# esi-neuroscience/syncopy

Hardware: AMD Instinct MI355X
Metric: trials/sec for mtmfft+coherence (256 ch x 4096 samples, 7 DPSS tapers, full CSD) (higher is better)
Workload: dtype f32 transforms; CSD operands fp16 hi+lo (22-bit), f32 accumulate; 1 GPU; BASELINE configs[2]: connectivityanalysis method='coh', AR(2) AnalogData, 256 ch x 4096 samp x 1000 trials per GPU, tapsmofrq=1 Hz (7 DPSS tapers), polyremoval=0, output='abs', inputs resident in HBM; trials_per_gpu=1000, channels=256, samples=4096, tapers=7, freqs=2049, batch=1000, fft_kernel=mtmfft_quad_kernel<12, 2, 2, false> + seq_mean_kernel

## Files before the change

### syncopy_amd/csrc/csdh.hip

```cpp
#include "spy_common.h"
#include "csd_args.h"
#include "csdh_kernel.h"
#include "csdh_launch.h"

namespace spycsd {

int csdh_run(hipStream_t stream, const float2* spec, long long nrows, int F, float2* acc, const float* absmax, int* flags, int f0,
             int nf, bool phase_exact) {
    if (nf <= 0 || nrows <= 0) return 0;
    if (nrows > 0x7fffffffLL) { spy::set_error("csd_accumulate: more than 2^31 - 1 rows in one call"); return -1; }
    CsdhArgs a{};
    a.spec = spec; a.nrows = nrows; a.F = F; a.acc = acc; a.absmax = absmax; a.flags = flags; a.f0 = f0; a.nf = nf;
    a.rs = (long long)F * 256; a.fs = 256;
    SPY_HIP_CHECK(hipFuncSetAttribute(reinterpret_cast<const void*>(csdh_kernel), hipFuncAttributeMaxDynamicSharedMemorySize,
                                      CSDH_LDS_BYTES));
    hipLaunchKernelGGL(csdh_kernel, dim3((unsigned)nf), dim3(512), CSDH_LDS_BYTES, stream, a);
    SPY_HIP_CHECK(hipGetLastError());
    CsdArgs b{};
    b.spec = spec; b.nrows = nrows; b.F = F; b.C = 256; b.acc = acc;
    b.nt = 8; b.ntiles = M3_TILES_PER_F; b.nitems = (long long)F * M3_TILES_PER_F; b.cpad = 256;
    b.item_base = (long long)f0 * M3_TILES_PER_F; b.item_end = (long long)(f0 + nf) * M3_TILES_PER_F;
    b.only_flagged = flags;
    if (phase_exact) {
        auto k = csd3m_kernel<256, 8, true, false, true>;
        SPY_HIP_CHECK(hipFuncSetAttribute(reinterpret_cast<const void*>(k), hipFuncAttributeMaxDynamicSharedMemorySize, M3_LDS_BYTES));
        hipLaunchKernelGGL(k, dim3((unsigned)nf), dim3(512), M3_LDS_BYTES, stream, b);
    } else {
        auto k = csd3m_kernel<256, 8, true, false, false>;
        SPY_HIP_CHECK(hipFuncSetAttribute(reinterpret_cast<const void*>(k), hipFuncAttributeMaxDynamicSharedMemorySize, M3_LDS_BYTES));
        hipLaunchKernelGGL(k, dim3((unsigned)nf), dim3(512), M3_LDS_BYTES, stream, b);
    }
    SPY_HIP_CHECK(hipGetLastError());
    return 0;
}

int csdh_absmax(hipStream_t stream, const float2* spec, long long nvalues, int nchan, float* absmax) {
    if (nvalues <= 0) return 0;
    if (nchan & 1 || nchan > 512 || 512 % nchan != 0) { spy::set_error("csd range pass: %d channels", nchan); return -1; }
    hipLaunchKernelGGL(csdh_absmax_kernel, dim3(2048), dim3(256), 0, stream, reinterpret_cast<const float4*>(spec), nvalues / 2, nchan,
                       reinterpret_cast<unsigned*>(absmax));
    SPY_HIP_CHECK(hipGetLastError());
    return 0;
}

}
```

### syncopy_amd/csrc/csdh_kernel.h

```cpp
#pragma once
#include "csd3m_kernel.h"

#ifndef CSDH_FENCE
#define CSDH_FENCE 0x78f
#endif
#ifndef CSDH_S1
#define CSDH_S1 7
#define CSDH_S2 15
#endif

#ifndef CSDH_ABL
#define CSDH_ABL 0
#endif

#ifdef CSDH_STAMPS
#define CSDH_STAMP(k) do { if (blockIdx.x == 0 && c >= 20 && c < 24) { asm volatile("s_waitcnt lgkmcnt(0)" ::: "memory"); \
        const unsigned long long t__ = __builtin_readcyclecounter(); \
        if (lane == 0) a.stamps[((c - 20) * 8 + G) * 8 + (k)] = t__; } } while (0)
#else
#define CSDH_STAMP(k) do { } while (0)
#endif

namespace spycsd {

typedef _Float16 f16x8 __attribute__((ext_vector_type(8)));
typedef float f32x2 __attribute__((ext_vector_type(2)));

struct CsdhArgs {
    const float2* spec;
    long long nrows;
    int F;
    float2* acc;
    const float* absmax;
    int* flags;
    int f0;
    int nf;
    unsigned long long* stamps;
    long long rs, fs;
};

constexpr int CSDH_PLANE = 16 * 1024;
constexpr int CSDH_BUF = 4 * CSDH_PLANE;
constexpr int CSDH_LDS_BYTES = 2 * CSDH_BUF + 1024 + 16;
constexpr int CSDH_KROWS = 32;

template <int NT_ = 17>
struct HTabT {
    static constexpr int NT = NT_, ND = 2;
    struct Gen { int ta[8][NT], tb[8][NT]; };
    static constexpr Gen make() {
        constexpr int SQR[6] = {8, 8, 12, 12, 4, 12}, SQC[6] = {0, 4, 0, 4, 0, 8};
        constexpr int DG[8] = {0, 10, 2, 14, 6, 8, 4, 12};
        Gen g{};
        int n[8] = {};
        for (int w = 0; w < 6; ++w)
            for (int r = SQR[w]; r < SQR[w] + 4; ++r)
                for (int c = SQC[w]; c < SQC[w] + 4; ++c) {
                    const int o = (r == SQR[w] && c == SQC[w] + 3) ? 6 + (w & 1) : w;
                    g.ta[o][n[o]] = r; g.tb[o][n[o]] = c; ++n[o];
                }
        for (int w = 6; w < 8; ++w)
            for (int b = 8 * (w - 6); b < 8 * (w - 6) + 8; b += 4)
                for (int r = b; r < b + 4; ++r)
                    for (int c = b; c < r; ++c) { g.ta[w][n[w]] = r; g.tb[w][n[w]] = c; ++n[w]; }
        for (int w = 0; w < 8; ++w)
            for (int d = DG[w]; d < DG[w] + 2; ++d) { g.ta[w][n[w]] = d; g.tb[w][n[w]] = d; ++n[w]; }
        return g;
    }
    static constexpr Gen T = make();
    static constexpr int ta(int g, int t) { return T.ta[g][t]; }
    static constexpr int tb(int g, int t) { return T.tb[g][t]; }
    static constexpr bool diag(int g, int t) { return T.ta[g][t] == T.tb[g][t]; }
    static constexpr int didx(int g, int t) {
        int d = 0;
        for (int u = 0; u < t; ++u) d += diag(g, u) ? 1 : 0;
        return d;
    }
    static constexpr bool complete() {
        int seen[16][16] = {};
        for (int w = 0; w < 8; ++w) {
            int nd = 0;
            for (int t = 0; t < NT; ++t) {
                if (T.ta[w][t] < T.tb[w][t] || T.ta[w][t] > 15 || T.tb[w][t] < 0) return false;
                ++seen[T.ta[w][t]][T.tb[w][t]];
                nd += diag(w, t) ? 1 : 0;
            }
            if (nd != ND) return false;
        }
        for (int r = 0; r < 16; ++r)
            for (int c = 0; c <= r; ++c)
                if (seen[r][c] != 1) return false;
        return true;
    }
};
using HTab = HTabT<>;
static_assert(HTab::complete(), "the deal of K4h's sub-tiles");
static_assert(HTab::NT == M3Tab<256>::NT, "17 sub-tiles per wave in either deal");

template <int G>
struct HPlan {
    using TAB = HTab;
    static constexpr int NT = TAB::NT;
    struct P {
        int tile[NT];
        int ablk[NT], bblk[NT];
        int aslot[NT], bslot[NT];
        bool aload[NT], bload[NT];
        bool diag[NT], dinb[NT];
    };
    static constexpr bool column_only(int x) {
        bool col = false;
        for (int t = 0; t < NT; ++t) {
            if (TAB::diag(G, t)) continue;
            if (TAB::ta(G, t) == x) return false;
            col = col || TAB::tb(G, t) == x;
        }
        return col;
    }
    static constexpr P make() {
        P p{};
        int key[NT] = {};
        for (int t = 0; t < NT; ++t) {
            p.tile[t] = t;
            key[t] = (TAB::tb(G, t) >> 1) * 256 + TAB::ta(G, t) * 16 + TAB::tb(G, t);
        }
        for (int i = 1; i < NT; ++i)
            for (int j = i; j > 0 && key[j] < key[j - 1]; --j) {
                int k = key[j]; key[j] = key[j - 1]; key[j - 1] = k;
                int u = p.tile[j]; p.tile[j] = p.tile[j - 1]; p.tile[j - 1] = u;
            }
        int ac[2] = {-1, -1}, bc[2] = {-1, -1};
        int alast = 1, blast = 1;
        for (int s = 0; s < NT; ++s) {
            const int t = p.tile[s];
            const int x = TAB::ta(G, t), y = TAB::tb(G, t);
            p.ablk[s] = x;
            p.bblk[s] = y;
            p.diag[s] = x == y;
            p.dinb[s] = x == y && column_only(x);
            p.aslot[s] = alast; p.aload[s] = false;
            p.bslot[s] = blast; p.bload[s] = false;
            if (!p.dinb[s]) {
                if (ac[0] == x) { p.aslot[s] = 0; }
                else if (ac[1] == x) { p.aslot[s] = 1; }
                else { p.aslot[s] = 1 - alast; p.aload[s] = true; ac[1 - alast] = x; }
                alast = p.aslot[s];
            }
            if (!p.diag[s] || p.dinb[s]) {
                if (bc[0] == y) { p.bslot[s] = 0; }
                else if (bc[1] == y) { p.bslot[s] = 1; }
                else { p.bslot[s] = 1 - blast; p.bload[s] = true; bc[1 - blast] = y; }
                blast = p.bslot[s];
            }
        }
        return p;
    }
    static constexpr P T = make();
};

__device__ __forceinline__ int csdh_exponent(float absmax) {
    const int e = (int)((__float_as_uint(absmax) >> 23) & 0xffu);
    int k = 141 - e;
    return k > 127 ? 127 : k;
}

__device__ __forceinline__ void csdh_tile(const f16x8 (&X)[4], const f16x8 (&Y)[4], f32x4& re, f32x4& im) {
    __builtin_amdgcn_s_setprio(1);
    im = __builtin_amdgcn_mfma_f32_16x16x32_f16(X[2], Y[0], im, 0, 0, 0);
    im = __builtin_amdgcn_mfma_f32_16x16x32_f16(X[2], Y[1], im, 0, 0, 0);
    im = __builtin_amdgcn_mfma_f32_16x16x32_f16(X[3], Y[0], im, 0, 0, 0);
    re = __builtin_amdgcn_mfma_f32_16x16x32_f16(X[0], Y[0], re, 0, 0, 0);
    re = __builtin_amdgcn_mfma_f32_16x16x32_f16(X[0], Y[1], re, 0, 0, 0);
    re = __builtin_amdgcn_mfma_f32_16x16x32_f16(X[1], Y[0], re, 0, 0, 0);
    re = __builtin_amdgcn_mfma_f32_16x16x32_f16(X[2], Y[2], re, 0, 0, 0);
    re = __builtin_amdgcn_mfma_f32_16x16x32_f16(X[2], Y[3], re, 0, 0, 0);
    re = __builtin_amdgcn_mfma_f32_16x16x32_f16(X[3], Y[2], re, 0, 0, 0);
    if (!(CSDH_ABL & 32)) im = -im;
    im = __builtin_amdgcn_mfma_f32_16x16x32_f16(X[0], Y[2], im, 0, 0, 0);
    im = __builtin_amdgcn_mfma_f32_16x16x32_f16(X[0], Y[3], im, 0, 0, 0);
    im = __builtin_amdgcn_mfma_f32_16x16x32_f16(X[1], Y[2], im, 0, 0, 0);
    __builtin_amdgcn_s_setprio(0);
}

__device__ __forceinline__ void csdh_diag_tile(const f16x8 (&X)[4], f32x4& s, f32x4& p, f32x4& m) {
    __builtin_amdgcn_s_setprio(1);
    m = __builtin_amdgcn_mfma_f32_16x16x32_f16(X[2], X[0], m, 0, 0, 0);
    m = __builtin_amdgcn_mfma_f32_16x16x32_f16(X[2], X[1], m, 0, 0, 0);
    m = __builtin_amdgcn_mfma_f32_16x16x32_f16(X[3], X[0], m, 0, 0, 0);
    s = __builtin_amdgcn_mfma_f32_16x16x32_f16(X[0], X[0], s, 0, 0, 0);
    s = __builtin_amdgcn_mfma_f32_16x16x32_f16(X[2], X[2], s, 0, 0, 0);
    p = __builtin_amdgcn_mfma_f32_16x16x32_f16(X[0], X[1], p, 0, 0, 0);
    p = __builtin_amdgcn_mfma_f32_16x16x32_f16(X[2], X[3], p, 0, 0, 0);
    if (!(CSDH_ABL & 32)) m = -m;
    __builtin_amdgcn_s_setprio(0);
}

template <int G, int s>
__device__ __forceinline__ void csdh_step(const f16x8 (&A)[2][4], const f16x8 (&B)[2][4], f32x4 (&re)[HTab::NT], f32x4 (&im)[HTab::NT],
                                          f32x4 (&pd)[HTab::ND]) {
    using PL = HPlan<G>;
    constexpr int t = PL::T.tile[s];
    if constexpr (PL::T.diag[s]) {
        const f16x8(&X)[4] = PL::T.dinb[s] ? B[PL::T.bslot[s]] : A[PL::T.aslot[s]];
        csdh_diag_tile(X, re[t], pd[HTab::didx(G, t)], im[t]);
    } else {
        csdh_tile(A[PL::T.aslot[s]], B[PL::T.bslot[s]], re[t], im[t]);
    }
}

template <int G>
__device__ __forceinline__ void csdh_fold_diagonal(f32x4 (&re)[HTab::NT], f32x4 (&im)[HTab::NT], f32x4 (&pd)[HTab::ND], float* ts,
                                                   int lane) {
    const int l15 = lane & 15, lq = lane >> 4;
    auto transposed = [&](const f32x4& v) {
#pragma unroll
        for (int r = 0; r < 4; ++r) ts[(4 * lq + r) * 17 + l15] = v[r];
        __builtin_amdgcn_fence(__ATOMIC_RELEASE, "wavefront");
        __builtin_amdgcn_wave_barrier();
        __builtin_amdgcn_fence(__ATOMIC_ACQUIRE, "wavefront");
        f32x4 o;
#pragma unroll
        for (int r = 0; r < 4; ++r) o[r] = ts[l15 * 17 + 4 * lq + r];
        __builtin_amdgcn_fence(__ATOMIC_RELEASE, "wavefront");
        __builtin_amdgcn_wave_barrier();
        __builtin_amdgcn_fence(__ATOMIC_ACQUIRE, "wavefront");
        return o;
    };
    m3_for<0, HTab::NT>([&](auto tc) {
        constexpr int t = decltype(tc)::value;
        if constexpr (HTab::diag(G, t)) {
            constexpr int d = HTab::didx(G, t);
            const f32x4 st = transposed(re[t]), pt = transposed(pd[d]), mt = transposed(im[t]);
#pragma unroll
            for (int r = 0; r < 4; ++r) {
                re[t][r] = 0.5f * (re[t][r] + st[r]) + (pd[d][r] + pt[r]);
                im[t][r] = im[t][r] - mt[r];
            }
        }
    });
}

template <int G, class KEXP>
__device__ __forceinline__ void csdh_finish(const CsdhArgs& a, f32x4 (&re)[HTab::NT], f32x4 (&im)[HTab::NT], f32x4 (&pd)[HTab::ND],
                                            float* ts, int nchunk, int f, int lane, int* vword, KEXP kexp) {
    using TAB = HTab;
    constexpr int NT = TAB::NT;
    const int l15 = lane & 15, lq = lane >> 4;
    const long long nrows = a.nrows;
    csdh_fold_diagonal<G>(re, im, pd, ts, lane);
    const float isign = (nchunk & 1) ? -1.f : 1.f;

    {
        const float floor2 = (float)nrows * 0.015625f;
        bool bad = false;
        m3_for<0, NT>([&](auto tc) {
            constexpr int t = decltype(tc)::value;
            if constexpr (TAB::diag(G, t)) {
                const bool dead = a.absmax[TAB::ta(G, t) * 16 + l15] == 0.f;
#pragma unroll
                for (int r = 0; r < 4; ++r)
                    if (4 * lq + r == l15) {
                        const float v = re[t][r];
                        bad = bad || !((v >= floor2 && v < __builtin_inff()) || (v == 0.f && dead));
                    }
            }
        });
        if (__any(bad) && lane == 0) *vword = 0;
    }
    __syncthreads();
    const bool valid = *vword != 0;
    if (a.flags && G == 0 && lane == 0) a.flags[f] = valid ? 0 : 1;
    if (!valid) return;

    m3_for<0, NT>([&](auto tc) {
        constexpr int t = decltype(tc)::value;
        constexpr int bi = TAB::ta(G, t), bj = TAB::tb(G, t);
        static_assert(bi >= bj, "a sub-tile lies on or below the diagonal");
        float2* const pb = a.acc + (size_t)f * 65536 + (size_t)(bi * 16 + 4 * lq) * 256 + bj * 16 + l15;
        const int kj = kexp(bj * 16 + l15);
        float2 old[4];
#pragma unroll
        for (int r = 0; r < 4; ++r) old[r] = pb[(size_t)r * 256];
#pragma unroll
        for (int r = 0; r < 4; ++r) {
            const int kk = -(kexp(bi * 16 + 4 * lq + r) + kj);
            pb[(size_t)r * 256] = make_float2(old[r].x + ldexpf(re[t][r], kk), old[r].y + ldexpf(isign * im[t][r], kk));
        }
    });
}

template <int G>
__device__ __forceinline__ void csdh_wave(const CsdhArgs& a, char* lds, int f, int lane) {
    using TAB = HTab;
    using PL = HPlan<G>;
    constexpr int NT = TAB::NT, ND = TAB::ND;
    constexpr int KG = G >> 1, CHH = G & 1;
    const int l15 = lane & 15, lq = lane >> 4;
    int* const kexp = reinterpret_cast<int*>(lds + 2 * CSDH_BUF);
    int* const vword = reinterpret_cast<int*>(lds + 2 * CSDH_BUF + 1024);

    const int lc0 = 128 * CHH + lane, lc1 = lc0 + 64;
    const int k0 = csdh_exponent(a.absmax[lc0]), k1 = csdh_exponent(a.absmax[lc1]);
    const float s0 = __uint_as_float((unsigned)(k0 + 127) << 23), s1 = __uint_as_float((unsigned)(k1 + 127) << 23);
    if (KG == 0) { kexp[lc0] = k0; kexp[lc1] = k1; }
    if (G == 0 && lane == 0) *vword = 1;

    const long long nrows = a.nrows;
    const int nchunk = (int)((nrows + CSDH_KROWS - 1) / CSDH_KROWS);
    const size_t rowstride = (size_t)a.rs;

    f32x2 st[8];
    const int nrows_i = (int)nrows;
    const int nfull = nrows_i / CSDH_KROWS;
    const char* const gb = reinterpret_cast<const char*>(a.spec) + ((size_t)f * a.fs + 128 * CHH) * 8;
    const size_t rowbytes = rowstride * 8;
    const unsigned voff = (unsigned)lane * 8u;
    const char* nextp = gb + (size_t)(CSDH_KROWS + 8 * KG) * rowbytes;
    auto fetch = [&](int c, int ph) {
        if (c < nfull) {
#pragma unroll
            for (int i = 0; i < 8; ++i) {
                if (CSDH_ABL & 1) st[i] = f32x2{(float)(i + lane), (float)(c - lane)};
                else if ((CSDH_ABL & 128) && c > 2) asm volatile("" : "+v"(st[i]));
                else {
                    typedef const __attribute__((address_space(1))) char gchar;
                    typedef const __attribute__((address_space(1))) f32x2 gf32x2;
                    gchar* rowp = (gchar*)(nextp + i * rowbytes);
                    asm("" : "+s"(rowp));
                    st[i] = *(gf32x2*)(rowp + voff + 512 * ph);
                }
            }
        } else {
            const int r0 = c * CSDH_KROWS + 8 * KG;
#pragma unroll
            for (int i = 0; i < 8; ++i) {
                const int r = min(r0 + i, nrows_i - 1);
                st[i] = *reinterpret_cast<const f32x2*>(gb + (size_t)r * rowbytes + 512 * ph + voff);
            }
        }
    };
    auto split2 = [](float x0, float x1, float s, unsigned& hi, unsigned& lo) {
        asm("v_fma_mixlo_f16 %0, %2, %4, 0\n\t"
            "v_fma_mixhi_f16 %0, %3, %4, 0\n\t"
            "v_fma_mixlo_f16 %1, %2, %4, -%0 op_sel_hi:[0,0,1]\n\t"
            "v_fma_mixhi_f16 %1, %3, %4, -%0 op_sel:[0,0,1] op_sel_hi:[0,0,1]"
            : "=&v"(hi), "=&v"(lo)
            : "v"(x0), "v"(x1), "v"(s));
    };
    typedef unsigned u32x4 __attribute__((ext_vector_type(4)));
    auto convert = [&](int c, int ph) {
        const float sc = ph ? s1 : s0;
        u32x4 rh, rl, ih, il;
        if (CSDH_ABL & 2) {
#pragma unroll
            for (int i = 0; i < 4; ++i) { rh[i] = rl[i] = __float_as_uint(st[2 * i][0]); ih[i] = il[i] = __float_as_uint(st[2 * i + 1][1]); }
        } else if (c < nfull) {
#pragma unroll
            for (int i = 0; i < 4; ++i) {
                unsigned h, l;
                split2(st[2 * i][0], st[2 * i + 1][0], sc, h, l);
                rh[i] = h; rl[i] = l;
                split2(st[2 * i][1], st[2 * i + 1][1], sc, h, l);
                ih[i] = h; il[i] = l;
            }
        } else {
            const int r0 = c * CSDH_KROWS + 8 * KG;
#pragma unroll
            for (int i = 0; i < 4; ++i) {
                const float sa = (r0 + 2 * i < nrows_i) ? sc : 0.f, sb = (r0 + 2 * i + 1 < nrows_i) ? sc : 0.f;
                unsigned h0, l0, h1, l1;
                split2(st[2 * i][0], st[2 * i][1], sa, h0, l0);
                split2(st[2 * i + 1][0], st[2 * i + 1][1], sb, h1, l1);
                rh[i] = (h0 & 0xffffu) | (h1 << 16);
                rl[i] = (l0 & 0xffffu) | (l1 << 16);
                ih[i] = (h0 >> 16) | (h1 & 0xffff0000u);
                il[i] = (l0 >> 16) | (l1 & 0xffff0000u);
            }
        }
        const int odd = c & 1;
        char* const w = lds + odd * CSDH_BUF + KG * 4096 + (lc0 + 64 * ph) * 16;
        char* const wr = w + (odd ? 2 * CSDH_PLANE : 0);
        char* const wi = w + (odd ? 0 : 2 * CSDH_PLANE);
        if (CSDH_ABL & 4) {
            if (rh[0] + rl[1] + ih[2] + il[3] == 123456u) *reinterpret_cast<u32x4*>(wr) = rh;
            return;
        }
        *reinterpret_cast<u32x4*>(wr) = rh;
        *reinterpret_cast<u32x4*>(wr + CSDH_PLANE) = rl;
        *reinterpret_cast<u32x4*>(wi) = ih;
        *reinterpret_cast<u32x4*>(wi + CSDH_PLANE) = il;
    };

    f32x4 re[NT], im[NT], pd[ND];
#pragma unroll
    for (int t = 0; t < NT; ++t)
#pragma unroll
        for (int r = 0; r < 4; ++r) { re[t][r] = 0.f; im[t][r] = 0.f; }
#pragma unroll
    for (int d = 0; d < ND; ++d)
#pragma unroll
        for (int r = 0; r < 4; ++r) pd[d][r] = 0.f;

    nextp -= (size_t)CSDH_KROWS * rowbytes;
    fetch(0, 0);
    convert(0, 0);
    fetch(0, 1);
    convert(0, 1);
    nextp += (size_t)CSDH_KROWS * rowbytes;
    __syncthreads();

    f16x8 A[2][4], B[2][4];
    unsigned rb = (unsigned)(lq * 4096 + l15 * 16);
    bool nofrag = false;
    auto ldfrag = [&](f16x8 (&dst)[4], int blk) {
#pragma unroll
        for (int p = 0; p < 4; ++p) {
            if (CSDH_ABL & 8) {
                asm volatile("" : "+v"(dst[p]));
                continue;
            }
            if ((CSDH_ABL & 64) && nofrag) continue;
            dst[p] = *reinterpret_cast<const f16x8*>(lds + rb + p * CSDH_PLANE + blk * 256);
        }
    };
    constexpr int S1 = CSDH_S1, S2 = CSDH_S2;

    for (int c = 0; c < nchunk; ++c) {
        CSDH_STAMP(0);
        if constexpr (PL::T.aload[0]) ldfrag(A[PL::T.aslot[0]], PL::T.ablk[0]);
        if constexpr (PL::T.bload[0]) ldfrag(B[PL::T.bslot[0]], PL::T.bblk[0]);
        fetch(c + 1, 0);
        __builtin_amdgcn_sched_barrier(CSDH_FENCE);
        m3_for<0, NT>([&](auto sc) {
            constexpr int s = decltype(sc)::value;
            if constexpr (s + 1 < NT) {
                if constexpr (PL::T.aload[s + 1]) ldfrag(A[PL::T.aslot[s + 1]], PL::T.ablk[s + 1]);
                if constexpr (PL::T.bload[s + 1]) ldfrag(B[PL::T.bslot[s + 1]], PL::T.bblk[s + 1]);
            }
            csdh_step<G, s>(A, B, re, im, pd);
            if constexpr (s == S1) {
                CSDH_STAMP(2);
#ifdef CSDH_STAMPS
                asm volatile("s_waitcnt vmcnt(0)" ::: "memory");
#endif
                CSDH_STAMP(3);
                convert(c + 1, 0);
                fetch(c + 1, 1);
                __builtin_amdgcn_sched_barrier(CSDH_FENCE);
                CSDH_STAMP(4);
            }
            if constexpr (s == 0) CSDH_STAMP(1);
            if constexpr (s == S2) {
                CSDH_STAMP(5);
#ifdef CSDH_STAMPS
                asm volatile("s_waitcnt vmcnt(0)" ::: "memory");
#endif
                CSDH_STAMP(6);
                convert(c + 1, 1);
            }
        });
        CSDH_STAMP(7);
        if (!(CSDH_ABL & 16)) __syncthreads();
        if (CSDH_ABL & 64) nofrag = true;
        rb ^= (unsigned)CSDH_BUF;
        nextp += (size_t)CSDH_KROWS * rowbytes;
    }

    csdh_finish<G>(a, re, im, pd, reinterpret_cast<float*>(lds + G * 2048), nchunk, f, lane, vword, [&](int ch) { return kexp[ch]; });
}

template <int G0, int G1>
__device__ __forceinline__ void csdh_dispatch(int g, const CsdhArgs& a, char* lds, int f, int lane) {
    if constexpr (G0 + 1 == G1) {
        csdh_wave<G0>(a, lds, f, lane);
    } else {
        constexpr int GM = (G0 + G1) / 2;
        if (g < GM) csdh_dispatch<G0, GM>(g, a, lds, f, lane);
        else csdh_dispatch<GM, G1>(g, a, lds, f, lane);
    }
}

__global__ void __launch_bounds__(512) SPY_M3_KATTR(8) csdh_kernel(CsdhArgs a) {
    SPY_DYN_SMEM(char, lds);
    const int tid = threadIdx.x;
    const int lane = tid & 63;
    const int wave = __builtin_amdgcn_readfirstlane(tid >> 6);
    const int f = a.f0 + (int)blockIdx.x;
    csdh_dispatch<0, 8>(wave, a, lds, f, lane);
}

__global__ void __launch_bounds__(256) csdh_absmax_kernel(const float4* __restrict__ spec, long long nquads, int C,
                                                          unsigned* __restrict__ out) {
    __shared__ unsigned sm[512];
    for (int i = threadIdx.x; i < 512; i += 256) sm[i] = 0u;
    __syncthreads();
    const long long per = C / 2;
    const long long stride = (long long)gridDim.x * 256;
    float m0 = 0.f, m1 = 0.f;
    long long q = (long long)blockIdx.x * 256 + threadIdx.x;
    const int cp = (int)(q % per);
    for (; q < nquads; q += stride) {
        const float4 v = spec[q];
        m0 = fmaxf(m0, fmaxf(fabsf(v.x), fabsf(v.y)));
        m1 = fmaxf(m1, fmaxf(fabsf(v.z), fabsf(v.w)));
    }
    atomicMax(&sm[2 * cp], __float_as_uint(m0));
    atomicMax(&sm[2 * cp + 1], __float_as_uint(m1));
    __syncthreads();
    for (int i = threadIdx.x; i < C; i += 256)
        if (sm[i]) atomicMax(&out[i], sm[i]);
}

}
```

Before: 51450 trials/s.

## Split CSD waves into heavy MFMA waves and loader waves with interleaved conversion

The sub-tile deal across the 8 waves changes. Four heavy waves now run only MFMA sub-tiles (22 each) at raised priority. The other four waves take fewer sub-tiles plus the diagonal blocks, and they also do all global fetches and fp16 hi/lo conversion, which are split into small pieces and interleaved between individual MFMAs. The fetch uses 16-byte vector loads with deeper prefetch (two chunks ahead), so spectra must now be 16-byte aligned. The aim is to keep the matrix pipes busy in some waves while the load and convert latency is hidden in the others, at the cost of load imbalance and higher register pressure in the loader waves.

```diff
diff --git a/syncopy_amd/csrc/csdh.hip b/syncopy_amd/csrc/csdh.hip
--- a/syncopy_amd/csrc/csdh.hip
+++ b/syncopy_amd/csrc/csdh.hip
@@ -9,6 +9,7 @@
              int nf, bool phase_exact) {
     if (nf <= 0 || nrows <= 0) return 0;
     if (nrows > 0x7fffffffLL) { spy::set_error("csd_accumulate: more than 2^31 - 1 rows in one call"); return -1; }
+    if (reinterpret_cast<uintptr_t>(spec) & 15u) { spy::set_error("csd_accumulate: 256-channel spectra must be 16-byte aligned"); return -1; }
     CsdhArgs a{};
     a.spec = spec; a.nrows = nrows; a.F = F; a.acc = acc; a.absmax = absmax; a.flags = flags; a.f0 = f0; a.nf = nf;
     a.rs = (long long)F * 256; a.fs = 256;
diff --git a/syncopy_amd/csrc/csdh_kernel.h b/syncopy_amd/csrc/csdh_kernel.h
--- a/syncopy_amd/csrc/csdh_kernel.h
+++ b/syncopy_amd/csrc/csdh_kernel.h
@@ -4,9 +4,14 @@
 #ifndef CSDH_FENCE
 #define CSDH_FENCE 0x78f
 #endif
-#ifndef CSDH_S1
-#define CSDH_S1 7
-#define CSDH_S2 15
+#ifndef CSDH_NH
+#define CSDH_NH 22
+#endif
+#ifndef CSDH_HEAVY_HI
+#define CSDH_HEAVY_HI 0
+#endif
+#ifndef CSDH_PRIO
+#define CSDH_PRIO 1
 #endif
 
 #ifndef CSDH_ABL
@@ -17,7 +22,10 @@
 #define CSDH_STAMP(k) do { if (blockIdx.x == 0 && c >= 20 && c < 24) { asm volatile("s_waitcnt lgkmcnt(0)" ::: "memory"); \
         const unsigned long long t__ = __builtin_readcyclecounter(); \
         if (lane == 0) a.stamps[((c - 20) * 8 + G) * 8 + (k)] = t__; } } while (0)
+#define CSDH_STAMP_HWID() do { if (blockIdx.x == 0 && lane == 0) \
+        a.stamps[256 + G] = __builtin_amdgcn_s_getreg(4 | (31 << 11)); } while (0)
 #else
+#define CSDH_STAMP_HWID() do { } while (0)
 #define CSDH_STAMP(k) do { } while (0)
 #endif
 
@@ -44,27 +52,36 @@
 constexpr int CSDH_LDS_BYTES = 2 * CSDH_BUF + 1024 + 16;
 constexpr int CSDH_KROWS = 32;
 
-template <int NT_ = 17>
+template <int NH_ = CSDH_NH>
 struct HTabT {
-    static constexpr int NT = NT_, ND = 2;
-    struct Gen { int ta[8][NT], tb[8][NT]; };
+    static constexpr int NH = NH_, NLO = 30 - NH_, NDL = 4;
+    static constexpr int NTMAX = NH > NLO + NDL ? NH : NLO + NDL;
+    static_assert(NH >= 17 && NH <= 24 && (96 - 4 * NH) % 4 == 0, "the heavy runs come out of the 96 full-row sub-tiles");
+    static constexpr bool heavy(int g) { return CSDH_HEAVY_HI ? g >= 4 : g < 4; }
+    static constexpr int idx(int g) { return g & 3; }
+    static constexpr int nt(int g) { return heavy(g) ? NH : NLO + NDL; }
+    static constexpr int nd(int g) { return heavy(g) ? 0 : NDL; }
+    struct Gen { int ta[8][NTMAX], tb[8][NTMAX]; };
     static constexpr Gen make() {
-        constexpr int SQR[6] = {8, 8, 12, 12, 4, 12}, SQC[6] = {0, 4, 0, 4, 0, 8};
-        constexpr int DG[8] = {0, 10, 2, 14, 6, 8, 4, 12};
+        int sr[96] = {}, sc[96] = {};
+        int m = 0;
+        for (int s = 0; s < 3; ++s)
+            for (int r = 4 * (s + 1); r < 16; ++r)
+                for (int c = 4 * s; c < 4 * s + 4; ++c) { sr[m] = r; sc[m] = c; ++m; }
         Gen g{};
-        int n[8] = {};
-        for (int w = 0; w < 6; ++w)
-            for (int r = SQR[w]; r < SQR[w] + 4; ++r)
-                for (int c = SQC[w]; c < SQC[w] + 4; ++c) {
-                    const int o = (r == SQR[w] && c == SQC[w] + 3) ? 6 + (w & 1) : w;
-                    g.ta[o][n[o]] = r; g.tb[o][n[o]] = c; ++n[o];
-                }
-        for (int w = 6; w < 8; ++w)
-            for (int b = 8 * (w - 6); b < 8 * (w - 6) + 8; b += 4)
-                for (int r = b; r < b + 4; ++r)
-                    for (int c = b; c < r; ++c) { g.ta[w][n[w]] = r; g.tb[w][n[w]] = c; ++n[w]; }
-        for (int w = 0; w < 8; ++w)
-            for (int d = DG[w]; d < DG[w] + 2; ++d) { g.ta[w][n[w]] = d; g.tb[w][n[w]] = d; ++n[w]; }
+        constexpr int per = (96 - 4 * NH) / 4;
+        for (int w = 0; w < 8; ++w) {
+            const int i = idx(w);
+            int n = 0;
+            if (heavy(w)) {
+                for (int k = 0; k < NH; ++k) { g.ta[w][n] = sr[i * NH + k]; g.tb[w][n] = sc[i * NH + k]; ++n; }
+            } else {
+                for (int k = 0; k < per; ++k) { g.ta[w][n] = sr[4 * NH + i * per + k]; g.tb[w][n] = sc[4 * NH + i * per + k]; ++n; }
+                for (int r = 4 * i; r < 4 * i + 4; ++r)
+                    for (int c = 4 * i; c < r; ++c) { g.ta[w][n] = r; g.tb[w][n] = c; ++n; }
+                for (int d = 4 * i; d < 4 * i + 4; ++d) { g.ta[w][n] = d; g.tb[w][n] = d; ++n; }
+            }
+        }
         return g;
     }
     static constexpr Gen T = make();
@@ -79,13 +96,14 @@
     static constexpr bool complete() {
         int seen[16][16] = {};
         for (int w = 0; w < 8; ++w) {
-            int nd = 0;
-            for (int t = 0; t < NT; ++t) {
+            int nd_ = 0;
+            for (int t = 0; t < nt(w); ++t) {
                 if (T.ta[w][t] < T.tb[w][t] || T.ta[w][t] > 15 || T.tb[w][t] < 0) return false;
                 ++seen[T.ta[w][t]][T.tb[w][t]];
-                nd += diag(w, t) ? 1 : 0;
-            }
-            if (nd != ND) return false;
+                nd_ += diag(w, t) ? 1 : 0;
+            }
+            if (nd_ != nd(w)) return false;
+            if (w < 4 && heavy(w) == heavy(w + 4)) return false;
         }
         for (int r = 0; r < 16; ++r)
             for (int c = 0; c <= r; ++c)
@@ -95,12 +113,11 @@
 };
 using HTab = HTabT<>;
 static_assert(HTab::complete(), "the deal of K4h's sub-tiles");
-static_assert(HTab::NT == M3Tab<256>::NT, "17 sub-tiles per wave in either deal");
 
 template <int G>
 struct HPlan {
     using TAB = HTab;
-    static constexpr int NT = TAB::NT;
+    static constexpr int NT = TAB::nt(G);
     struct P {
         int tile[NT];
         int ablk[NT], bblk[NT];
@@ -164,53 +181,68 @@
     return k > 127 ? 127 : k;
 }
 
-__device__ __forceinline__ void csdh_tile(const f16x8 (&X)[4], const f16x8 (&Y)[4], f32x4& re, f32x4& im) {
-    __builtin_amdgcn_s_setprio(1);
+__device__ __forceinline__ void csdh_tile_begin() { __builtin_amdgcn_sched_barrier(0); if (!CSDH_PRIO) __builtin_amdgcn_s_setprio(1); }
+__device__ __forceinline__ void csdh_tile_end() { if (!CSDH_PRIO) __builtin_amdgcn_s_setprio(0); __builtin_amdgcn_sched_barrier(0); }
+struct CsdhNoWork { __device__ __forceinline__ void operator()(int) const {} };
+
+template <class W>
+__device__ __forceinline__ void csdh_tile(const f16x8 (&X)[4], const f16x8 (&Y)[4], f32x4& re, f32x4& im, W&& work) {
+    csdh_tile_begin();
     im = __builtin_amdgcn_mfma_f32_16x16x32_f16(X[2], Y[0], im, 0, 0, 0);
+    work(0);
     im = __builtin_amdgcn_mfma_f32_16x16x32_f16(X[2], Y[1], im, 0, 0, 0);
     im = __builtin_amdgcn_mfma_f32_16x16x32_f16(X[3], Y[0], im, 0, 0, 0);
     re = __builtin_amdgcn_mfma_f32_16x16x32_f16(X[0], Y[0], re, 0, 0, 0);
+    work(1);
     re = __builtin_amdgcn_mfma_f32_16x16x32_f16(X[0], Y[1], re, 0, 0, 0);
     re = __builtin_amdgcn_mfma_f32_16x16x32_f16(X[1], Y[0], re, 0, 0, 0);
     re = __builtin_amdgcn_mfma_f32_16x16x32_f16(X[2], Y[2], re, 0, 0, 0);
+    work(2);
     re = __builtin_amdgcn_mfma_f32_16x16x32_f16(X[2], Y[3], re, 0, 0, 0);
     re = __builtin_amdgcn_mfma_f32_16x16x32_f16(X[3], Y[2], re, 0, 0, 0);
     if (!(CSDH_ABL & 32)) im = -im;
     im = __builtin_amdgcn_mfma_f32_16x16x32_f16(X[0], Y[2], im, 0, 0, 0);
+    work(3);
     im = __builtin_amdgcn_mfma_f32_16x16x32_f16(X[0], Y[3], im, 0, 0, 0);
     im = __builtin_amdgcn_mfma_f32_16x16x32_f16(X[1], Y[2], im, 0, 0, 0);
-    __builtin_amdgcn_s_setprio(0);
-}
-
-__device__ __forceinline__ void csdh_diag_tile(const f16x8 (&X)[4], f32x4& s, f32x4& p, f32x4& m) {
-    __builtin_amdgcn_s_setprio(1);
+    csdh_tile_end();
+}
+
+template <class W>
+__device__ __forceinline__ void csdh_diag_tile(const f16x8 (&X)[4], f32x4& s, f32x4& p, f32x4& m, W&& work) {
+    csdh_tile_begin();
     m = __builtin_amdgcn_mfma_f32_16x16x32_f16(X[2], X[0], m, 0, 0, 0);
+    work(0);
     m = __builtin_amdgcn_mfma_f32_16x16x32_f16(X[2], X[1], m, 0, 0, 0);
     m = __builtin_amdgcn_mfma_f32_16x16x32_f16(X[3], X[0], m, 0, 0, 0);
+    work(1);
     s = __builtin_amdgcn_mfma_f32_16x16x32_f16(X[0], X[0], s, 0, 0, 0);
     s = __builtin_amdgcn_mfma_f32_16x16x32_f16(X[2], X[2], s, 0, 0, 0);
+    work(2);
     p = __builtin_amdgcn_mfma_f32_16x16x32_f16(X[0], X[1], p, 0, 0, 0);
+    work(3);
     p = __builtin_amdgcn_mfma_f32_16x16x32_f16(X[2], X[3], p, 0, 0, 0);
     if (!(CSDH_ABL & 32)) m = -m;
-    __builtin_amdgcn_s_setprio(0);
-}
-
-template <int G, int s>
-__device__ __forceinline__ void csdh_step(const f16x8 (&A)[2][4], const f16x8 (&B)[2][4], f32x4 (&re)[HTab::NT], f32x4 (&im)[HTab::NT],
-                                          f32x4 (&pd)[HTab::ND]) {
+    csdh_tile_end();
+}
+
+constexpr int csdh_npd(int g) { return HTab::nd(g) ? HTab::nd(g) : 1; }
+template <int G, int s, class W = CsdhNoWork>
+__device__ __forceinline__ void csdh_step(const f16x8 (&A)[2][4], const f16x8 (&B)[2][4], f32x4 (&re)[HTab::nt(G)],
+                                          f32x4 (&im)[HTab::nt(G)], f32x4 (&pd)[csdh_npd(G)], W&& work = W()) {
     using PL = HPlan<G>;
     constexpr int t = PL::T.tile[s];
     if constexpr (PL::T.diag[s]) {
         const f16x8(&X)[4] = PL::T.dinb[s] ? B[PL::T.bslot[s]] : A[PL::T.aslot[s]];
-        csdh_diag_tile(X, re[t], pd[HTab::didx(G, t)], im[t]);
+        csdh_diag_tile(X, re[t], pd[HTab::didx(G, t)], im[t], work);
     } else {
-        csdh_tile(A[PL::T.aslot[s]], B[PL::T.bslot[s]], re[t], im[t]);
+        csdh_tile(A[PL::T.aslot[s]], B[PL::T.bslot[s]], re[t], im[t], work);
     }
 }
 
 template <int G>
-__device__ __forceinline__ void csdh_fold_diagonal(f32x4 (&re)[HTab::NT], f32x4 (&im)[HTab::NT], f32x4 (&pd)[HTab::ND], float* ts,
-                                                   int lane) {
+__device__ __forceinline__ void csdh_fold_diagonal(f32x4 (&re)[HTab::nt(G)], f32x4 (&im)[HTab::nt(G)], f32x4 (&pd)[csdh_npd(G)],
+                                                   float* ts, int lane) {
     const int l15 = lane & 15, lq = lane >> 4;
     auto transposed = [&](const f32x4& v) {
 #pragma unroll
@@ -226,7 +258,7 @@
         __builtin_amdgcn_fence(__ATOMIC_ACQUIRE, "wavefront");
         return o;
     };
-    m3_for<0, HTab::NT>([&](auto tc) {
+    m3_for<0, HTab::nt(G)>([&](auto tc) {
         constexpr int t = decltype(tc)::value;
         if constexpr (HTab::diag(G, t)) {
             constexpr int d = HTab::didx(G, t);
@@ -241,10 +273,10 @@
 }
 
 template <int G, class KEXP>
-__device__ __forceinline__ void csdh_finish(const CsdhArgs& a, f32x4 (&re)[HTab::NT], f32x4 (&im)[HTab::NT], f32x4 (&pd)[HTab::ND],
-                                            float* ts, int nchunk, int f, int lane, int* vword, KEXP kexp) {
+__device__ __forceinline__ void csdh_finish(const CsdhArgs& a, f32x4 (&re)[HTab::nt(G)], f32x4 (&im)[HTab::nt(G)],
+                                            f32x4 (&pd)[csdh_npd(G)], float* ts, int nchunk, int f, int lane, int* vword, KEXP kexp) {
     using TAB = HTab;
-    constexpr int NT = TAB::NT;
+    constexpr int NT = TAB::nt(G);
     const int l15 = lane & 15, lq = lane >> 4;
     const long long nrows = a.nrows;
     csdh_fold_diagonal<G>(re, im, pd, ts, lane);
@@ -289,124 +321,148 @@
     });
 }
 
+constexpr int csdh_cpoint(int nt, int ph) { return ((2 * ph + 1) * nt) / 8; }
+constexpr int csdh_cphase(int nt, int s) {
+    for (int ph = 0; ph < 4; ++ph)
+        if (csdh_cpoint(nt, ph) == s) return ph;
+    return -1;
+}
+
 template <int G>
 __device__ __forceinline__ void csdh_wave(const CsdhArgs& a, char* lds, int f, int lane) {
     using TAB = HTab;
     using PL = HPlan<G>;
-    constexpr int NT = TAB::NT, ND = TAB::ND;
-    constexpr int KG = G >> 1, CHH = G & 1;
+    constexpr int NT = TAB::nt(G), NPD = csdh_npd(G);
+    constexpr bool LOADER = !TAB::heavy(G);
+    constexpr int KG = TAB::idx(G);
     const int l15 = lane & 15, lq = lane >> 4;
     int* const kexp = reinterpret_cast<int*>(lds + 2 * CSDH_BUF);
     int* const vword = reinterpret_cast<int*>(lds + 2 * CSDH_BUF + 1024);
-
-    const int lc0 = 128 * CHH + lane, lc1 = lc0 + 64;
-    const int k0 = csdh_exponent(a.absmax[lc0]), k1 = csdh_exponent(a.absmax[lc1]);
-    const float s0 = __uint_as_float((unsigned)(k0 + 127) << 23), s1 = __uint_as_float((unsigned)(k1 + 127) << 23);
-    if (KG == 0) { kexp[lc0] = k0; kexp[lc1] = k1; }
+    CSDH_STAMP_HWID();
+
+    float sc00 = 0.f, sc01 = 0.f, sc10 = 0.f, sc11 = 0.f;
+    if constexpr (LOADER) {
+        const int k00 = csdh_exponent(a.absmax[2 * lane]), k01 = csdh_exponent(a.absmax[2 * lane + 1]);
+        const int k10 = csdh_exponent(a.absmax[128 + 2 * lane]), k11 = csdh_exponent(a.absmax[129 + 2 * lane]);
+        sc00 = __uint_as_float((unsigned)(k00 + 127) << 23); sc01 = __uint_as_float((unsigned)(k01 + 127) << 23);
+        sc10 = __uint_as_float((unsigned)(k10 + 127) << 23); sc11 = __uint_as_float((unsigned)(k11 + 127) << 23);
+        if (KG == 0) { kexp[2 * lane] = k00; kexp[2 * lane + 1] = k01; kexp[128 + 2 * lane] = k10; kexp[129 + 2 * lane] = k11; }
+    }
     if (G == 0 && lane == 0) *vword = 1;
 
     const long long nrows = a.nrows;
     const int nchunk = (int)((nrows + CSDH_KROWS - 1) / CSDH_KROWS);
     const size_t rowstride = (size_t)a.rs;
 
-    f32x2 st[8];
+    f32x4 stg[2][4];
     const int nrows_i = (int)nrows;
     const int nfull = nrows_i / CSDH_KROWS;
-    const char* const gb = reinterpret_cast<const char*>(a.spec) + ((size_t)f * a.fs + 128 * CHH) * 8;
+    const char* const gb = reinterpret_cast<const char*>(a.spec) + (size_t)f * a.fs * 8;
     const size_t rowbytes = rowstride * 8;
-    const unsigned voff = (unsigned)lane * 8u;
-    const char* nextp = gb + (size_t)(CSDH_KROWS + 8 * KG) * rowbytes;
-    auto fetch = [&](int c, int ph) {
+    const unsigned voff = (unsigned)lane * 16u;
+    const char* nextp = gb + (size_t)(8 * KG) * rowbytes;
+    auto fetch = [&](const char* cp, int c, int ph) {
+        f32x4(&st)[4] = stg[ph & 1];
+        const int rh = ph >> 1, ch = ph & 1;
         if (c < nfull) {
 #pragma unroll
-            for (int i = 0; i < 8; ++i) {
-                if (CSDH_ABL & 1) st[i] = f32x2{(float)(i + lane), (float)(c - lane)};
+            for (int i = 0; i < 4; ++i) {
+                if (CSDH_ABL & 1) st[i] = f32x4{(float)(i + lane), (float)(c - lane), (float)(i - lane), (float)(c + lane)};
                 else if ((CSDH_ABL & 128) && c > 2) asm volatile("" : "+v"(st[i]));
                 else {
                     typedef const __attribute__((address_space(1))) char gchar;
-                    typedef const __attribute__((address_space(1))) f32x2 gf32x2;
-                    gchar* rowp = (gchar*)(nextp + i * rowbytes);
+                    typedef const __attribute__((address_space(1))) f32x4 gf32x4;
+                    gchar* rowp = (gchar*)(cp + (4 * rh + i) * rowbytes);
                     asm("" : "+s"(rowp));
-                    st[i] = *(gf32x2*)(rowp + voff + 512 * ph);
+                    st[i] = *(gf32x4*)(rowp + voff + 1024 * ch);
                 }
             }
         } else {
-            const int r0 = c * CSDH_KROWS + 8 * KG;
-#pragma unroll
-            for (int i = 0; i < 8; ++i) {
-                const int r = min(r0 + i, nrows_i - 1);
-                st[i] = *reinterpret_cast<const f32x2*>(gb + (size_t)r * rowbytes + 512 * ph + voff);
-            }
-        }
-    };
-    auto split2 = [](float x0, float x1, float s, unsigned& hi, unsigned& lo) {
-        asm("v_fma_mixlo_f16 %0, %2, %4, 0\n\t"
-            "v_fma_mixhi_f16 %0, %3, %4, 0\n\t"
-            "v_fma_mixlo_f16 %1, %2, %4, -%0 op_sel_hi:[0,0,1]\n\t"
-            "v_fma_mixhi_f16 %1, %3, %4, -%0 op_sel:[0,0,1] op_sel_hi:[0,0,1]"
-            : "=&v"(hi), "=&v"(lo)
-            : "v"(x0), "v"(x1), "v"(s));
-    };
-    typedef unsigned u32x4 __attribute__((ext_vector_type(4)));
-    auto convert = [&](int c, int ph) {
-        const float sc = ph ? s1 : s0;
-        u32x4 rh, rl, ih, il;
+            const long long r0 = (long long)c * CSDH_KROWS + 8 * KG + 4 * rh;
+#pragma unroll
+            for (int i = 0; i < 4; ++i) {
+                const long long r = r0 + i < nrows ? r0 + i : nrows - 1;
+                st[i] = *reinterpret_cast<const f32x4*>(gb + (size_t)r * rowbytes + 1024 * ch + voff);
+            }
+        }
+    };
+    typedef unsigned u32x2 __attribute__((ext_vector_type(2)));
+    u32x2 cv[2][4];
+    auto piece = [&](int c, int ph, int j) {
+        const f32x4(&st)[4] = stg[ph & 1];
+        const int rhalf = ph >> 1, ch = ph & 1, k = j >> 1, i = j & 1;
+        const float sc = ch == 0 ? (k == 0 ? sc00 : sc01) : (k == 0 ? sc10 : sc11);
+        float sa = sc, sb = sc;
+        if (c >= nfull) {
+            const long long r0 = (long long)c * CSDH_KROWS + 8 * KG + 4 * rhalf + 2 * i;
+            sa = r0 < nrows ? sc : 0.f;
+            sb = r0 + 1 < nrows ? sc : 0.f;
+        }
+        unsigned rh, rl, ih, il;
         if (CSDH_ABL & 2) {
-#pragma unroll
-            for (int i = 0; i < 4; ++i) { rh[i] = rl[i] = __float_as_uint(st[2 * i][0]); ih[i] = il[i] = __float_as_uint(st[2 * i + 1][1]); }
-        } else if (c < nfull) {
-#pragma unroll
-            for (int i = 0; i < 4; ++i) {
-                unsigned h, l;
-                split2(st[2 * i][0], st[2 * i + 1][0], sc, h, l);
-                rh[i] = h; rl[i] = l;
-                split2(st[2 * i][1], st[2 * i + 1][1], sc, h, l);
-                ih[i] = h; il[i] = l;
-            }
+            rh = rl = __float_as_uint(st[2 * i][2 * k]); ih = il = __float_as_uint(st[2 * i + 1][2 * k + 1]);
         } else {
-            const int r0 = c * CSDH_KROWS + 8 * KG;
-#pragma unroll
-            for (int i = 0; i < 4; ++i) {
-                const float sa = (r0 + 2 * i < nrows_i) ? sc : 0.f, sb = (r0 + 2 * i + 1 < nrows_i) ? sc : 0.f;
-                unsigned h0, l0, h1, l1;
-                split2(st[2 * i][0], st[2 * i][1], sa, h0, l0);
-                split2(st[2 * i + 1][0], st[2 * i + 1][1], sb, h1, l1);
-                rh[i] = (h0 & 0xffffu) | (h1 << 16);
-                rl[i] = (l0 & 0xffffu) | (l1 << 16);
-                ih[i] = (h0 >> 16) | (h1 & 0xffff0000u);
-                il[i] = (l0 >> 16) | (l1 & 0xffff0000u);
-            }
-        }
+            asm("v_fma_mixlo_f16 %0, %4, %8, 0\n\t"
+                "v_fma_mixlo_f16 %2, %6, %8, 0\n\t"
+                "v_fma_mixhi_f16 %0, %5, %9, 0\n\t"
+                "v_fma_mixhi_f16 %2, %7, %9, 0\n\t"
+                "v_fma_mixlo_f16 %1, %4, %8, -%0 op_sel_hi:[0,0,1]\n\t"
+                "v_fma_mixlo_f16 %3, %6, %8, -%2 op_sel_hi:[0,0,1]\n\t"
+                "v_fma_mixhi_f16 %1, %5, %9, -%0 op_sel:[0,0,1] op_sel_hi:[0,0,1]\n\t"
+                "v_fma_mixhi_f16 %3, %7, %9, -%2 op_sel:[0,0,1] op_sel_hi:[0,0,1]"
+                : "=&v"(rh), "=&v"(rl), "=&v"(ih), "=&v"(il)
+                : "v"(st[2 * i][2 * k]), "v"(st[2 * i + 1][2 * k]), "v"(st[2 * i][2 * k + 1]), "v"(st[2 * i + 1][2 * k + 1]), "v"(sa), "v"(sb));
+        }
+        cv[k][0][i] = rh; cv[k][1][i] = rl; cv[k][2][i] = ih; cv[k][3][i] = il;
+    };
+    auto flush = [&](int c, int ph) {
+        const int rhalf = ph >> 1, ch = ph & 1;
         const int odd = c & 1;
-        char* const w = lds + odd * CSDH_BUF + KG * 4096 + (lc0 + 64 * ph) * 16;
+        char* const w = lds + odd * CSDH_BUF + KG * 4096 + (128 * ch + 2 * lane) * 16 + 8 * rhalf;
         char* const wr = w + (odd ? 2 * CSDH_PLANE : 0);
         char* const wi = w + (odd ? 0 : 2 * CSDH_PLANE);
-        if (CSDH_ABL & 4) {
-            if (rh[0] + rl[1] + ih[2] + il[3] == 123456u) *reinterpret_cast<u32x4*>(wr) = rh;
-            return;
-        }
-        *reinterpret_cast<u32x4*>(wr) = rh;
-        *reinterpret_cast<u32x4*>(wr + CSDH_PLANE) = rl;
-        *reinterpret_cast<u32x4*>(wi) = ih;
-        *reinterpret_cast<u32x4*>(wi + CSDH_PLANE) = il;
-    };
-
-    f32x4 re[NT], im[NT], pd[ND];
+#pragma unroll
+        for (int k = 0; k < 2; ++k) {
+            if (CSDH_ABL & 4) {
+                if (cv[k][0][0] + cv[k][1][1] + cv[k][2][0] + cv[k][3][1] == 123456u) *reinterpret_cast<u32x2*>(wr) = cv[k][0];
+                continue;
+            }
+            *reinterpret_cast<u32x2*>(wr + 16 * k) = cv[k][0];
+            *reinterpret_cast<u32x2*>(wr + 16 * k + CSDH_PLANE) = cv[k][1];
+            *reinterpret_cast<u32x2*>(wi + 16 * k) = cv[k][2];
+            *reinterpret_cast<u32x2*>(wi + 16 * k + CSDH_PLANE) = cv[k][3];
+        }
+    };
+    auto convert = [&](int c, int ph) {
+#pragma unroll
+        for (int j = 0; j < 4; ++j) piece(c, ph, j);
+        flush(c, ph);
+    };
+
+    f32x4 re[NT], im[NT], pd[NPD];
 #pragma unroll
     for (int t = 0; t < NT; ++t)
 #pragma unroll
         for (int r = 0; r < 4; ++r) { re[t][r] = 0.f; im[t][r] = 0.f; }
 #pragma unroll
-    for (int d = 0; d < ND; ++d)
+    for (int d = 0; d < NPD; ++d)
 #pragma unroll
         for (int r = 0; r < 4; ++r) pd[d][r] = 0.f;
 
-    nextp -= (size_t)CSDH_KROWS * rowbytes;
-    fetch(0, 0);
-    convert(0, 0);
-    fetch(0, 1);
-    convert(0, 1);
-    nextp += (size_t)CSDH_KROWS * rowbytes;
+    if constexpr (LOADER) {
+        fetch(nextp, 0, 0);
+        fetch(nextp, 0, 1);
+        convert(0, 0);
+        fetch(nextp, 0, 2);
+        convert(0, 1);
+        fetch(nextp, 0, 3);
+        convert(0, 2);
+        convert(0, 3);
+        nextp += (size_t)CSDH_KROWS * rowbytes;
+        fetch(nextp, 1, 0);
+        fetch(nextp, 1, 1);
+        __builtin_amdgcn_sched_barrier(CSDH_FENCE);
+    }
     __syncthreads();
 
     f16x8 A[2][4], B[2][4];
@@ -423,48 +479,58 @@
             dst[p] = *reinterpret_cast<const f16x8*>(lds + rb + p * CSDH_PLANE + blk * 256);
         }
     };
-    constexpr int S1 = CSDH_S1, S2 = CSDH_S2;
-
+    static_assert(csdh_cpoint(NT, 0) < csdh_cpoint(NT, 1) && csdh_cpoint(NT, 1) < csdh_cpoint(NT, 2) &&
+                  csdh_cpoint(NT, 2) < csdh_cpoint(NT, 3) && csdh_cpoint(NT, 3) < NT, "four conversion points in the walk");
+
+    if (CSDH_PRIO && !LOADER) __builtin_amdgcn_s_setprio(1);
     for (int c = 0; c < nchunk; ++c) {
         CSDH_STAMP(0);
         if constexpr (PL::T.aload[0]) ldfrag(A[PL::T.aslot[0]], PL::T.ablk[0]);
         if constexpr (PL::T.bload[0]) ldfrag(B[PL::T.bslot[0]], PL::T.bblk[0]);
-        fetch(c + 1, 0);
-        __builtin_amdgcn_sched_barrier(CSDH_FENCE);
         m3_for<0, NT>([&](auto sc) {
             constexpr int s = decltype(sc)::value;
             if constexpr (s + 1 < NT) {
                 if constexpr (PL::T.aload[s + 1]) ldfrag(A[PL::T.aslot[s + 1]], PL::T.ablk[s + 1]);
                 if constexpr (PL::T.bload[s + 1]) ldfrag(B[PL::T.bslot[s + 1]], PL::T.bblk[s + 1]);
             }
-            csdh_step<G, s>(A, B, re, im, pd);
-            if constexpr (s == S1) {
-                CSDH_STAMP(2);
-#ifdef CSDH_STAMPS
-                asm volatile("s_waitcnt vmcnt(0)" ::: "memory");
-#endif
-                CSDH_STAMP(3);
-                convert(c + 1, 0);
-                fetch(c + 1, 1);
-                __builtin_amdgcn_sched_barrier(CSDH_FENCE);
-                CSDH_STAMP(4);
+            constexpr int cph = LOADER ? csdh_cphase(NT, s) : -1;
+            if constexpr (cph < 0) {
+                csdh_step<G, s>(A, B, re, im, pd);
+            } else {
+                if constexpr (cph == 0) CSDH_STAMP(2);
+                if constexpr (cph == 3) CSDH_STAMP(5);
+                csdh_step<G, s>(A, B, re, im, pd, [&](int j) {
+                    __builtin_amdgcn_sched_barrier(0);
+                    piece(c + 1, cph, j);
+                    __builtin_amdgcn_sched_barrier(0);
+                });
             }
             if constexpr (s == 0) CSDH_STAMP(1);
-            if constexpr (s == S2) {
-                CSDH_STAMP(5);
-#ifdef CSDH_STAMPS
-                asm volatile("s_waitcnt vmcnt(0)" ::: "memory");
-#endif
-                CSDH_STAMP(6);
-                convert(c + 1, 1);
+            if constexpr (LOADER) {
+                m3_for<0, 4>([&](auto pc) {
+                    constexpr int ph = decltype(pc)::value;
+                    if constexpr (s == csdh_cpoint(NT, ph)) {
+                        if constexpr (ph == 0) CSDH_STAMP(3);
+                        flush(c + 1, ph);
+                        if constexpr (ph < 2) {
+                            fetch(nextp, c + 1, ph + 2);
+                        } else {
+                            if constexpr (ph == 2) nextp += (size_t)CSDH_KROWS * rowbytes;
+                            fetch(nextp, c + 2, ph - 2);
+                        }
+                        __builtin_amdgcn_sched_barrier(CSDH_FENCE);
+                        if constexpr (ph == 0) CSDH_STAMP(4);
+                        if constexpr (ph == 3) CSDH_STAMP(6);
+                    }
+                });
             }
         });
         CSDH_STAMP(7);
         if (!(CSDH_ABL & 16)) __syncthreads();
         if (CSDH_ABL & 64) nofrag = true;
         rb ^= (unsigned)CSDH_BUF;
-        nextp += (size_t)CSDH_KROWS * rowbytes;
-    }
+    }
+    if (CSDH_PRIO && !LOADER) __builtin_amdgcn_s_setprio(0);
 
     csdh_finish<G>(a, re, im, pd, reinterpret_cast<float*>(lds + G * 2048), nchunk, f, lane, vword, [&](int ch) { return kexp[ch]; });
 }
```

After: 52280 trials/s (median of 6 runs). 1.02x the previous value.
